# 0xPolygonZero/proof-protocol-decoder

Measured on AMD Instinct MI355X. Metric: txn-proofs/sec (whole node), 256-txn synthetic block, higher is better.
Workload: dtype u64 (Goldilocks field)

## Files before the change

### include/bpg.h

```cpp
#ifndef BPG_H
#define BPG_H
#include <stddef.h>
#include <stdint.h>

#ifdef __cplusplus
extern "C" {
#endif

typedef enum {
  BP_OK = 0,
  BP_ERR_ABORTED = -1,
  BP_ERR_INVALID_INPUT = -2,
  BP_ERR_RANGE = -3,
  BP_ERR_DEVICE = -4,
  BP_ERR_VERIFY = -5,
  BP_ERR_UNSUPPORTED = -6
} bp_status;

const char* bp_last_error(void);
const char* bp_version(void);
int bp_device_count(void);
int bp_use_blocking_sync(int device);
int bp_host_wait_mode(int device);

// ... 4 lines not shown
enum { BP_NTT_FWD_BR2NAT = 0, BP_NTT_INV_NAT2BR = 1, BP_NTT_FWD_NAT = 2, BP_NTT_INV_NAT = 3 };
int bp_ntt_batch(uint64_t* d_cols, uint32_t log_n, uint32_t n_cols, uint64_t col_stride, int dir,
                 void* stream);

int bp_intt_batch(const uint64_t* d_values, uint64_t in_stride, uint64_t* d_coeffs_out, uint64_t out_stride,
                  uint32_t log_n, uint32_t n_cols, void* stream);

int bp_lde_batch(const uint64_t* d_in, uint64_t in_stride, uint64_t* d_coeffs_out, uint64_t coeffs_stride,
                 uint64_t* d_lde_out, uint64_t lde_stride, uint32_t log_n, uint32_t rate_bits,
                 uint32_t n_cols, int from_coeffs, void* stream);

int bp_debug_copy_u64(const uint64_t* d_in, uint64_t* d_out, uint64_t n, void* stream);

int bp_debug_field_ops(const uint64_t* d_a, const uint64_t* d_b, uint64_t* d_out, uint64_t n, void* stream);
int bp_debug_lazy_forms(const uint64_t* d_a, const uint64_t* d_b, uint64_t* d_out, uint64_t n, void* stream);
int bp_debug_mul_pow2(const uint64_t* d_a, uint64_t* d_out, uint64_t n, void* stream);

void bp_tune_quad_threshold(uint64_t n_perms);
void bp_tune_merkle_fused(int mode);
void bp_tune_merkle_wide(int log2_parents);
void bp_tune_poseidon_mx(int on);
void bp_tune_poseidon_mx_sets(int sets);
void bp_tune_poseidon_grouped(int on);
void bp_tune_assume_loaded(int mode);
void bp_tune_rec_batch(int n);
void bp_tune_side_lanes(int n);
void bp_tune_rec_riders(int on);
void bp_tune_txn_group(int n);
void bp_tune_rec_group(int mode);
int bp_debug_rec_batch_histogram(uint64_t* out, uint32_t n, int reset);
// ... 343 lines not shown
```

### proof_protocol_decoder_amd/_abi.py

```python
import ctypes as C
from ctypes import POINTER as P

vp, cp, i, sz, dbl = C.c_void_p, C.c_char_p, C.c_int, C.c_size_t, C.c_double
u8, u32, u64, i32, i64 = C.c_uint8, C.c_uint32, C.c_uint64, C.c_int32, C.c_int64
u8p, u32p, u64p, i32p, szp = P(u8), P(u32), P(u64), P(i32), P(sz)
u8pp = P(u8p)

BP_OK, BP_ERR_ABORTED, BP_ERR_INVALID_INPUT, BP_ERR_RANGE, BP_ERR_DEVICE, BP_ERR_VERIFY, BP_ERR_UNSUPPORTED = 0, -1, -2, -3, -4, -5, -6
STATUS_NAMES = {v: k for k, v in list(globals().items()) if k == "BP_OK" or k.startswith("BP_ERR_")}
BP_SET_SKIP_LINK_CHECK = 1
BP_NUM_TABLES, BP_IR_WORDS, BP_PV_WORDS = 7, 25, 13

KNOBS = ("quad_threshold", "assume_loaded", "merkle_fused", "merkle_wide", "poseidon_mx", "poseidon_mx_sets",
         "poseidon_grouped", "ntt_mx", "ntt_split", "k5_spread", "host_wait", "host_poseidon", "rec_batch",
         "witness_threads", "side_lanes")


def _u32s(*names):
    return [(n, u32) for n in names]


class AirFamily(C.Structure):
    _fields_ = _u32s("first_index", "count", "kind", "degree")

# ... 105 lines not shown
_trace = (i, [vp, u64, u32, vp, vp])
_check = [u32, _cfg, vp, u64, vp, u64p, u32, u64p, u32p, P(AirViolation), u32, u32p]
_knob, _ir_flag, _buf = (None, [i]), (i, [u64p, i]), [u8pp, szp]
PROTOTYPES = {
    "bp_last_error": (cp, []),
    "bp_version": (cp, []),
    "bp_device_count": (i, []),
    "bp_use_blocking_sync": (i, [i]),
    "bp_host_wait_mode": (i, [i]),
    "bp_ntt_batch": (i, [vp, u32, u32, u64, i, vp]),
    "bp_intt_batch": (i, [vp, u64, vp, u64, u32, u32, vp]),
    "bp_lde_batch": (i, [vp, u64, vp, u64, vp, u64, u32, u32, u32, i, vp]),
    "bp_debug_copy_u64": (i, [vp, vp, u64, vp]),
    "bp_debug_field_ops": (i, [vp, vp, vp, u64, vp]),
    "bp_debug_lazy_forms": (i, [vp, vp, vp, u64, vp]),
    "bp_debug_mul_pow2": (i, [vp, vp, u64, vp]),
    "bp_tune_quad_threshold": (None, [u64]),
    "bp_tune_merkle_fused": _knob,
    "bp_tune_merkle_wide": _knob,
    "bp_tune_poseidon_mx": _knob,
    "bp_tune_poseidon_mx_sets": _knob,
    "bp_tune_poseidon_grouped": _knob,
    "bp_tune_assume_loaded": _knob,
    "bp_tune_rec_batch": _knob,
    "bp_tune_side_lanes": _knob,
    "bp_tune_rec_riders": _knob,
    "bp_tune_txn_group": _knob,
    "bp_tune_rec_group": _knob,
    "bp_debug_rec_batch_histogram": (i, [u64p, u32, i]),
    "bp_tune_witness_threads": _knob,
# ... 119 lines not shown
```

### proof_protocol_decoder_amd/csrc/air.hpp

```cpp
#pragma once
#include <cstdint>
#include <type_traits>
#include "gl.hpp"
#if defined(__HIP__)
#include "poseidon.cuh"
#endif

namespace bpg {
namespace air {

constexpr uint32_t SYNTHETIC = 0, KECCAK_F = 1, LOGIC = 2, MEMORY = 3, ARITHMETIC = 4, BYTE_PACKING = 5, KECCAK_SPONGE = 6, ARITHMETIC_MUL = 7, PLONK = 8, COUNT = 9;

struct Shape {
  uint32_t air_id, n_cols, n_const, deg_pow;
};

template <class T>
struct Ops;

#if defined(__HIP__)
template <>
struct Ops<uint64_t> {
  typedef uint64_t T;
  static __device__ __forceinline__ T k(uint64_t c) { return c; }
// ... 654 lines not shown
    out.all(U4 + k, F::sub(F::add(F::mul(m, conv), cin), F::add(p, F::mul(F::k(65536), c))));
    cin = c;
  }
  if (u == 7) out.all(U5, cin);
}
}

namespace plonk {
constexpr uint32_t N_COLS = 135, N_CONST = 85, N_ROUTED = 80, N_SLOTS = 20, N_SBOX = 11, N_CONSTRAINTS = 213, N_UNITS = 11;
constexpr uint32_t CST_ARITH = 0, CST_SBOX = 1, CST_C0 = 2, CST_C1 = 3, CST_HASH = 4, CST_SIGMA = 5;
constexpr uint32_t COL_SBOX = 80;
constexpr uint32_t G0 = 0, G1 = 20, G2 = 64, G3 = 86, G4 = 90, G5 = 208;
constexpr uint32_t HASH_ROW0 = 4, HASH_ROWS_MAX = 13, ZERO_ROW = 1, MAX_PI = 8 * HASH_ROWS_MAX;
constexpr uint32_t MERKLE_ROW0 = HASH_ROW0 + HASH_ROWS_MAX, MERKLE_ROWS_MAX = 96, MERKLE_ZERO_COL = 79, LEAF_ROWS_MAX = 120;
constexpr uint32_t H_IN = 0, H_OUT = 12, H_FULL1 = 24, H_PART = 60, H_FULL2 = 82, H_SWAP = 130, H_DELTA = 131, H_WIRES = 135;
struct Layout {
  uint32_t pi_len, n_paths, depth, path_pi0, leaf_len = 0;
};
GL_HD uint32_t hash_rows(uint32_t pi_len) { return (pi_len + 7) / 8; }
GL_HD uint32_t merkle_rows(const Layout& L) { return L.n_paths * L.depth; }
GL_HD uint32_t leaf_rows(const Layout& L) { return L.leaf_len ? L.n_paths * hash_rows(L.leaf_len) : 0; }
GL_HD uint32_t leaf_row0(const Layout& L) { return MERKLE_ROW0 + merkle_rows(L); }
GL_HD uint32_t arith_row0(const Layout& L) { return (MERKLE_ROW0 + merkle_rows(L) + leaf_rows(L) + 3) & ~3u; }
GL_HD bool layout_ok(const Layout& L, uint32_t n) {
  return L.pi_len >= 1 && L.pi_len <= MAX_PI && merkle_rows(L) <= MERKLE_ROWS_MAX && (L.n_paths == 0 || L.depth >= 1) &&
         L.path_pi0 + 8 * L.n_paths <= L.pi_len && (L.leaf_len == 0 || (L.leaf_len > 8 && L.n_paths >= 1)) &&
         leaf_rows(L) <= LEAF_ROWS_MAX && arith_row0(L) + 4 <= n;
}
GL_HD bool hash_word_is_carried(uint32_t pi_len, uint32_t h, uint32_t k) {
  const uint32_t H = hash_rows(pi_len), last = pi_len - 8 * (H - 1);
// ... 596 lines not shown
```

### proof_protocol_decoder_amd/csrc/prover.cpp

```cpp
#include <cstdio>
#include <cstdlib>
#include "prover.hpp"
#include "tune.hpp"
#include <algorithm>
#include <chrono>
#if defined(__x86_64__)
#include <immintrin.h>
#endif
#include <memory>
#include <mutex>
#include <unordered_map>
#include <thread>

namespace bpg {

static const uint64_t RC_HOST[360] = {
#include "poseidon_rc.inc"
};
static inline uint64_t sbox_host(uint64_t x) {
  uint64_t x2 = gl::mulc(x, x), x4 = gl::mulc(x2, x2), x3 = gl::mulc(x2, x);
  return gl::mulc(x3, x4);
}
static const uint32_t MDS_C[12] = {17, 15, 41, 16, 2, 28, 13, 13, 39, 18, 34, 20};
static inline void mds_finish_host(const uint64_t al[12], const uint64_t ah[12], uint64_t s[12]) {
// ... 514 lines not shown
                  int loaded, uint32_t batch) {
  QuotArgs& qa = *out;
  const uint32_t log_n = cfg.log_n, r = cfg.rate_bits, R = 1u << r, C = cfg.n_cols, K = cfg.n_const;
  const air::Shape shape{cfg.air_id, C, K, cfg.deg_pow};
  const uint32_t A = air::any_n_aux(shape);
  const uint64_t N = (uint64_t)1 << log_n, M = N << r;
  const uint64_t wM = gl::root(log_n + r), wN = gl::root(log_n);
  qa.trace_stride = qa.aux_stride = qa.const_stride = M;
  TRY(get_table(0, log_n, 0, &qa.tw_n));
  qa.air_id = cfg.air_id;
  qa.log_n = log_n; qa.rate_bits = r; qa.n_cols = C; qa.n_const = K; qa.n_aux = A; qa.deg_pow = cfg.deg_pow;
  qa.n_air_constraints = air::any_n_constraints(shape);
  qa.n_constraints = qa.n_air_constraints + air::any_n_ctl_constraints(shape);
  qa.side_rows = cfg.air_id == air::PLONK ? 1 : 0;
  qa.n_air_units = air::any_n_units(shape) - qa.side_rows;
  qa.aux_per_unit = cfg.air_id == air::SYNTHETIC ? std::max<uint32_t>(16, (A + 15) / 16) : A;
  qa.n_ctl_units = cfg.air_id == air::PLONK ? 0 : (A + qa.aux_per_unit - 1) / qa.aux_per_unit;
  qa.n_ports = air::prog::is_registered(cfg.air_id) && A > 1 ? A / 2 : 0;
  if (qa.n_ports) qa.n_ctl_units = qa.n_ports;
  const uint32_t n_units = qa.n_air_units + qa.n_ctl_units, wg_x = (uint32_t)((M + 255) / 256) * std::max<uint32_t>(1, batch);
  const uint32_t loaded_rows = (cfg.air_id == air::SYNTHETIC && !tune().k5_spread.load(std::memory_order_relaxed))
                                   ? 1 : std::min<uint32_t>(n_units, std::max<uint32_t>(1, (256 + wg_x - 1) / wg_x));
  const bool is_loaded = loaded < 0 ? device_loaded() : loaded != 0;
  const uint32_t want_rows = is_loaded ? loaded_rows : std::min<uint32_t>(n_units, std::max<uint32_t>(1, (2048 + wg_x - 1) / wg_x));
  qa.units_per_wg = (n_units + want_rows - 1) / want_rows;
  qa.alpha0 = alpha0; qa.alpha1 = alpha1;
  qa.g = wN; qa.g_inv = gl::inv(wN); qa.n_inv = gl::inv(N);
  if (coset)
    for (uint32_t t = 0; t < R; t++) {
      coset->g_t[t] = gl::mulc(gl::GENERATOR, gl::pow(wM, t));
// ... 414 lines not shown
```

### proof_protocol_decoder_amd/csrc/stark_api.cpp

```cpp
#include <algorithm>
#include <cstdlib>
#include <cstring>
#include <vector>
#include "caller_table.hpp"

using namespace bpg;

namespace {
constexpr uint32_t LONE_PI_LEN = 4;
void lone_public_input_list(uint64_t seed, uint64_t out[LONE_PI_LEN]) {
  for (uint64_t j = 0; j < LONE_PI_LEN; j++) {
    uint64_t z = (seed ^ ((0x50 + j) << 32)) + 0x9E3779B97F4A7C15ULL;
    z = (z ^ (z >> 30)) * 0xBF58476D1CE4E5B9ULL;
    z = (z ^ (z >> 27)) * 0x94D049BB133111EBULL;
    out[j] = gl::canon(z ^ (z >> 31));
  }
}
int prove_lone(Worker& w, const CallerTable& t, uint8_t** out, size_t* out_len) {
  Challenger ch;
  Committed consts, trace;
  const uint64_t* d_values = nullptr;
  int rc = commit_caller_table(w, ch, t, &consts, &trace, &d_values);
  if (rc) return rc;
  Ctl ctl;
// ... 3 lines not shown
  std::vector<uint64_t> proof;
  if ((rc = stark_prove(w, t.cfg, t.cfg.n_const ? &consts : nullptr, trace, d_values, ctl, ch, proof))) return rc;
  return emit(proof, out, out_len);
}
}

extern "C" {

void bp_free_buffer(uint8_t* buf) { std::free(buf); }
int bp_debug_poseidon_host(uint64_t* states, size_t n) try {
  if (!states && n) return bpg::fail(BP_ERR_INVALID_INPUT, "bp_debug_poseidon_host: null states");
  for (size_t i = 0; i < n; i++) bpg::poseidon_host(states + 12 * i);
  return BP_OK;
}
BPG_ABI_CATCH("bp_debug_poseidon_host")

void bp_release_cached_memory(void) { release_parked_workers(); }

int bp_stark_prove_air(uint32_t air_id, const bp_stark_cfg* cfg, uint64_t seed, uint64_t const_seed, int device,
                       uint8_t** out, size_t* out_len) try {
  if (!cfg || !out || !out_len) return fail(BP_ERR_INVALID_INPUT, "bp_stark_prove_air: null argument");
  if (air::prog::is_registered(air_id))
    return fail(BP_ERR_INVALID_INPUT, "bp_stark_prove_air: a registered AIR has no witness generator to draw from a seed: prove its trace "
                "with bp_stark_prove_trace");
  const StarkCfg c = to_cfg(*cfg, air_id);
  int rc = check_cfg(c);
  if (rc) return rc;
  const uint64_t N = (uint64_t)1 << c.log_n;
  WorkerLease lease(device, table_arena_bytes(c, false) + ARENA_SLACK);
  if (lease.rc()) return lease.rc();
// ... 415 lines not shown
```

### proof_protocol_decoder_amd/csrc/stark_kernels.hip

```cpp
#include "common.hpp"
#include "gl.hpp"
#include "poseidon.cuh"
#include "poseidon_mx.cuh"
#include "stark_kernels.hpp"
#include "arg_ring.hpp"
#include "quotient_dev.cuh"
#include "air_program.hpp"

namespace {

using gl::Ext;
using namespace bpg::k5;

__device__ __forceinline__ uint64_t splitmix64(uint64_t x) {
  uint64_t z = x + 0x9E3779B97F4A7C15ULL;
  z = (z ^ (z >> 30)) * 0xBF58476D1CE4E5B9ULL;
  z = (z ^ (z >> 27)) * 0x94D049BB133111EBULL;
  return z ^ (z >> 31);
}
__device__ __forceinline__ uint64_t rnd(uint64_t seed, uint64_t col, uint64_t row) {
  return gl::canon(splitmix64(seed ^ (col << 32) ^ row));
}
__device__ __forceinline__ uint64_t pow_e(uint64_t t, uint32_t e) {
  return e == 3 ? gl::mulc(gl::mulc(t, t), t) : t;
// ... 689 lines not shown
    aux[(uint64_t)(k + 1 < ct::PLONK_CHUNKS ? k + 1 : 0) * n] = P;
  }
}
__global__ void __launch_bounds__(256) plonk_partial_products_kernel(bpg::ArgPtr<bpg::AuxArgs> args, uint32_t log_n) {
  BPG_ARG_BATCH(bpg::AuxArgs, args);
  if (gridDim.x * gridDim.y * gridDim.z <= 64) __builtin_amdgcn_s_setprio(3);
  const bpg::AuxArgs& a = batch[blockIdx.z];
  const uint32_t n = 1u << log_n, i = blockIdx.x * blockDim.x + threadIdx.x, c = blockIdx.y / 9, k = 1 + blockIdx.y % 9;
  if (i >= n) return;
  const uint64_t z_next = a.aux[(uint64_t)(10 * c) * n + ((i + 1) & (n - 1))];
  uint64_t* p = a.aux + (uint64_t)(10 * c + k) * n + i;
  *p = gl::mulc(*p, z_next);
}

#ifndef BPG_PLONK_HASH_WAVES
#define BPG_PLONK_HASH_WAVES 2
#endif
template <uint32_t AIR>
__global__ void __launch_bounds__(256) __attribute__((amdgpu_waves_per_eu(AIR == bpg::air::KECCAK_F ? 3 : 1)))
quotient_air_kernel(bpg::ArgPtr<bpg::QuotArgs> args) {
  BPG_ARG_BATCH(bpg::QuotArgs, args);
  if (gridDim.x * gridDim.y * gridDim.z <= 64) __builtin_amdgcn_s_setprio(3);
  const bpg::QuotArgs& q = batch[blockIdx.z];
  const uint64_t rows = (uint64_t)1 << (q.log_n + q.rate_bits);
  const uint64_t pos = blockIdx.x * (uint64_t)blockDim.x + threadIdx.x;
  if (pos >= rows) return;
  const uint32_t n = 1u << q.log_n;
  const uint32_t t = (uint32_t)(pos >> q.log_n), m = (uint32_t)(pos & (n - 1));
  DevEmit out{q.apow, q.n_constraints, row_point(q, t, m),
              {gl::dot_zero(), gl::dot_zero(), gl::dot_zero(), gl::dot_zero()}, 0, 0, false};
  DevRow row{q.trace_lde, q.aux_lde, q.const_lde, q.trace_stride, q.aux_stride, q.const_stride, pos,
// ... 9 lines not shown
      const uint32_t k0 = (u - q.n_air_units) * q.aux_per_unit, k1 = min(k0 + q.aux_per_unit, q.n_aux);
      const bpg::air::Shape cs{AIR, q.n_cols, q.n_const, q.deg_pow};
      bpg::air::ctl::eval<uint64_t>(cs, q.n_air_constraints, k0, k1, q.ctl.v, row, out);
    }
  }
  const uint64_t r0 = out.result(0), r1 = out.result(1);
  if (gridDim.y == 1 && q.side_rows == 0) {
    const uint64_t zh_inv = q.apow[2 * (size_t)q.n_constraints + 32 + t];
    q.qvals[pos] = gl::mulc(r0, zh_inv);
    q.qvals[rows + pos] = gl::mulc(r1, zh_inv);
  } else {
    q.partial[((uint64_t)blockIdx.y * 2) * rows + pos] = r0;
    q.partial[((uint64_t)blockIdx.y * 2 + 1) * rows + pos] = r1;
  }
}
__global__ void __launch_bounds__(256) __attribute__((amdgpu_waves_per_eu(BPG_PLONK_HASH_WAVES)))
quotient_plonk_hash_kernel(bpg::ArgPtr<bpg::QuotArgs> args, uint32_t wg_row) {
  BPG_ARG_BATCH(bpg::QuotArgs, args);
  if (gridDim.x * gridDim.y * gridDim.z <= 64) __builtin_amdgcn_s_setprio(3);
  const bpg::QuotArgs& q = batch[blockIdx.z];
  const uint64_t rows = (uint64_t)1 << (q.log_n + q.rate_bits);
  const uint64_t pos = blockIdx.x * (uint64_t)blockDim.x + threadIdx.x;
  if (pos >= rows) return;
  const uint32_t n = 1u << q.log_n;
  const uint32_t t = (uint32_t)(pos >> q.log_n), m = (uint32_t)(pos & (n - 1));
  DevEmit out{q.apow, q.n_constraints, row_point(q, t, m),
              {gl::dot_zero(), gl::dot_zero(), gl::dot_zero(), gl::dot_zero()}, 0, 0, false};
  DevRow row{q.trace_lde, q.aux_lde, q.const_lde, q.trace_stride, q.aux_stride, q.const_stride, pos,
             ((uint64_t)t << q.log_n) | ((m + 1) & (n - 1)), out.rp.x, q.ctl.pub};
  bpg::air::plonk::eval_hash_unit<uint64_t, DevRow, DevEmit, false>(row, out);
  const uint64_t qh = row.cst(bpg::air::plonk::CST_HASH);
  q.partial[((uint64_t)wg_row * 2) * rows + pos] = gl::mulc(out.result(0), qh);
  q.partial[((uint64_t)wg_row * 2 + 1) * rows + pos] = gl::mulc(out.result(1), qh);
}
__global__ void __launch_bounds__(256) quotient_sum_kernel(bpg::ArgPtr<bpg::QuotArgs> args, uint32_t n_wg_rows) {
  BPG_ARG_BATCH(bpg::QuotArgs, args);
  if (gridDim.x * gridDim.y * gridDim.z <= 64) __builtin_amdgcn_s_setprio(3);
  const bpg::QuotArgs& q = batch[blockIdx.z];
  const uint64_t rows = (uint64_t)1 << (q.log_n + q.rate_bits);
  const uint64_t pos = blockIdx.x * (uint64_t)blockDim.x + threadIdx.x;
  if (pos >= rows) return;
  const uint32_t j = blockIdx.y, t = (uint32_t)(pos >> q.log_n);
  uint64_t acc = 0;
  for (uint32_t c = 0; c < n_wg_rows; c++) acc = gl::addc(acc, q.partial[((uint64_t)c * 2 + j) * rows + pos]);
  q.qvals[(uint64_t)j * rows + pos] = gl::mulc(acc, q.apow[2 * (size_t)q.n_constraints + 32 + t]);
}
struct CosetTab {
  uint64_t v[48];
};
struct AlphaTabArgs {
  uint64_t* out;
  uint64_t a0, a1;
};
__global__ void __launch_bounds__(256)
alpha_table_kernel(bpg::ArgPtr<AlphaTabArgs> args, uint32_t T, CosetTab ct) {
  BPG_ARG_BATCH(AlphaTabArgs, args);
  if (gridDim.x * gridDim.y * gridDim.z <= 64) __builtin_amdgcn_s_setprio(3);
  uint64_t* __restrict__ out = batch[blockIdx.z].out;
  const uint64_t a0 = batch[blockIdx.z].a0, a1 = batch[blockIdx.z].a1;
  const uint32_t e = blockIdx.x * blockDim.x + threadIdx.x;
  if (blockIdx.y == 0 && e < 48) out[2 * (uint64_t)T + e] = ct.v[e];
  if (e >= T) return;
  out[(uint64_t)blockIdx.y * T + e] = gl::pow(blockIdx.y ? a1 : a0, e);
}
__global__ void __launch_bounds__(256) quotient_chunks_kernel(bpg::ArgPtr<bpg::ChunkArgs> args) {
  BPG_ARG_BATCH(bpg::ChunkArgs, args);
  if (gridDim.x * gridDim.y * gridDim.z <= 64) __builtin_amdgcn_s_setprio(3);
  const bpg::ChunkArgs& c = batch[blockIdx.z];
  const uint32_t pos = blockIdx.x * blockDim.x + threadIdx.x, n = 1u << c.log_n;
  if (pos >= n) return;
  const uint32_t j = blockIdx.y, R = 1u << c.rate_bits;
  const uint64_t* e = c.e + (uint64_t)j * ((uint64_t)n << c.rate_bits);
  uint64_t d[16];
  for (uint32_t t = 0; t < R; t++) d[t] = gl::mulc(e[(uint64_t)t * n + pos], c.inv_scale[(uint64_t)t * n + pos]);
// ... 633 lines not shown
    BPG_LAUNCH_CHECK();
    plonk_partial_products_kernel<<<dim3(gx, 18, batch), 256, 0, st>>>(ab, log_n);
    BPG_LAUNCH_CHECK();
    return BP_OK;
  }
  const dim3 grid(n_aux - p0, 1, batch);
  const uint32_t reads = air_id < air::COUNT ? air::DESC[air_id].aux_reads : 0;
  KernelTimer kt(PROF_AUX, st, 8.0 * (double)((uint64_t)1 << log_n) * (reads + 1) * (n_aux - p0) * batch, true);
  air::dispatch(reads ? air_id : air::ARITHMETIC, [&](auto A) {
    if constexpr (air::DESC[A.value].aux_reads || A.value == air::ARITHMETIC)
      BPG_LAUNCH_TIMED(kt, aux_suffix_product_kernel<A.value>, grid, threads, 0, st, ab, log_n, n_cols);
  });
  BPG_LAUNCH_CHECK();
  return BP_OK;
}
int launch_quotient(const QuotArgs* qs, uint32_t batch, const QuotCoset& coset, hipStream_t st) {
  if (int rc = check_batch(batch)) return rc;
  const QuotArgs& q = qs[0];
  const uint64_t rows = (uint64_t)1 << (q.log_n + q.rate_bits);
  CosetTab ct;
  for (int t = 0; t < 16; t++) { ct.v[t] = coset.g_t[t]; ct.v[16 + t] = coset.zh_t[t]; ct.v[32 + t] = coset.zh_inv_t[t]; }
  AlphaTabArgs tabs[MAX_LOCKSTEP];
  for (uint32_t b = 0; b < batch; b++) tabs[b] = AlphaTabArgs{const_cast<uint64_t*>(qs[b].apow), qs[b].alpha0, qs[b].alpha1};
  BPG_ARG_BLOCKS(at, tabs, batch, st);
  alpha_table_kernel<<<dim3(ceil_div(q.n_constraints, 256), 2, batch), 256, 0, st>>>(at, q.n_constraints, ct);
  BPG_LAUNCH_CHECK();
  const uint32_t n_units = q.n_air_units + q.n_ctl_units, wg_rows = ceil_div(n_units, q.units_per_wg);
  BPG_ARG_BLOCKS(qb, qs, batch, st);
  if (q.n_ports)
    if (int rc = launch_beta_tables(qb_dev, batch, st)) return rc;
  dim3 g1(ceil_div(rows, 256), wg_rows, batch);
  KernelTimer kt(PROF_K5 + (q.air_id < air::COUNT ? q.air_id : 0), st, 8.0 * (double)rows * ((double)q.n_cols + q.n_aux + q.n_const + 2) * batch, true);
  if (bpg::air::prog::is_registered(q.air_id)) {
    if (int rc = launch_quotient_program(qb_dev, q, g1, kt, st)) return rc;
  } else air::dispatch(q.air_id, [&](auto A) { BPG_LAUNCH_TIMED(kt, quotient_air_kernel<A.value>, g1, 256, 0, st, qb); });
  kt.stop();
  if (q.side_rows) {
    BPG_LAUNCH_CHECK();
    KernelTimer kh(PROF_K5 + q.air_id, st, 0.0, true);
    BPG_LAUNCH_TIMED(kh, quotient_plonk_hash_kernel, dim3(ceil_div(rows, 256), 1, batch), 256, 0, st, qb, wg_rows);
  }
// ... 153 lines not shown
```

### proof_protocol_decoder_amd/csrc/stark_kernels.hpp

```cpp
#pragma once
#include <hip/hip_runtime.h>
#include <cstdint>
#include "air.hpp"
#include "gl.hpp"

namespace bpg {

struct Ctl {
  uint64_t v[4];
  uint64_t pub[4] = {0, 0, 0, 0};
};

constexpr uint32_t MAX_BATCH = 8;
constexpr uint32_t MAX_LOCKSTEP = 24;
int arg_ring_put(hipStream_t st, const void* blocks, size_t bytes, const void** dev);
template <class A>
using ArgPtr = const __attribute__((address_space(4))) A*;
template <class A>
inline ArgPtr<A> arg_ptr(const A* dev) { return (ArgPtr<A>)dev; }
#define BPG_ARG_BATCH(T, args) const T* __restrict__ batch = (const T*)(args)
template <class A>
inline int arg_put(hipStream_t st, const A* a, uint32_t n, const A** dev) {
  const void* d = nullptr;
  const int rc = arg_ring_put(st, a, sizeof(A) * n, &d);
// ... 2 lines not shown
}

struct QuotArgs {
  const uint64_t *trace_lde, *aux_lde, *const_lde;
  uint64_t trace_stride, aux_stride, const_stride;
  uint64_t *partial, *qvals;
  const uint64_t* tw_n;
  const uint64_t* apow;
  uint32_t air_id, log_n, rate_bits, n_cols, n_const, n_aux, deg_pow;
  uint32_t n_air_constraints, n_constraints, n_air_units, n_ctl_units, aux_per_unit, units_per_wg;
  uint32_t side_rows;
  uint32_t n_ports;
  uint64_t alpha0, alpha1, g, g_inv, n_inv;
  Ctl ctl;
};
inline size_t quotient_table_words(const QuotArgs& q) { return 2 * (size_t)q.n_constraints + 48 + (q.n_ports ? 256 : 0); }
struct QuotCoset {
  uint64_t g_t[16], zh_t[16], zh_inv_t[16];
};
struct SynthTraceArgs {
  uint64_t* trace;
  const uint64_t* consts;
  uint64_t seed;
};
struct AuxArgs {
  const uint64_t* trace;
  uint64_t* aux;
  Ctl ctl;
  const uint64_t* consts = nullptr;
};
struct PowerVecArgs {
// ... 116 lines not shown
int launch_aux(const AuxArgs* a, uint32_t batch, uint32_t air_id, uint32_t n_cols, uint32_t log_n, hipStream_t st);
int launch_plonk_constants(uint64_t* d_out, uint32_t log_n, uint64_t seed, const air::plonk::Layout& lay, hipStream_t st);
struct PlonkTraceArgs {
  uint64_t* trace;
  const uint64_t* consts;
  uint64_t seed, pub[4];
  const uint64_t* hash_rows;
  uint32_t n_hash_rows;
  uint32_t n_merkle_rows = 0, arith_row0 = (air::plonk::MERKLE_ROW0 + 3) & ~3u;
};
int launch_plonk_trace(const PlonkTraceArgs* a, uint32_t batch, uint32_t log_n, hipStream_t st);
int launch_quotient(const QuotArgs* q, uint32_t batch, const QuotCoset& coset, hipStream_t st);
inline int launch_quotient(const QuotArgs& q, const QuotCoset& coset, hipStream_t st) { return launch_quotient(&q, 1, coset, st); }
struct KernelTimer;
int launch_quotient_program(const QuotArgs* qb, const QuotArgs& q0, dim3 grid, KernelTimer& kt, hipStream_t st);
int launch_beta_tables(const QuotArgs* qb, uint32_t batch, hipStream_t st);
int launch_port_terms(const AuxArgs& a, uint32_t air_id, uint32_t log_n, uint64_t trace_stride, uint64_t* d_pole, hipStream_t st);
int launch_port_products(const AuxArgs* a, uint32_t batch, uint32_t air_id, uint32_t log_n, uint64_t trace_stride, hipStream_t st);
int launch_quotient_chunks(const ChunkArgs* c, uint32_t batch, hipStream_t st);
int launch_power_vectors(const PowerVecArgs* a, uint32_t batch, uint32_t log_n, uint32_t n_points, hipStream_t st);
inline int launch_power_vectors(uint64_t* d_out, uint32_t log_n, gl::Ext z0, gl::Ext z1, uint32_t n_points,
                                hipStream_t st, gl::Ext z2 = gl::Ext{1, 0}) {
  const PowerVecArgs a{d_out, {z0, z1, z2}};
  return launch_power_vectors(&a, 1, log_n, n_points, st);
}
int launch_alpha_pows(const AlphaPowArgs* a, uint32_t batch, uint32_t count, hipStream_t st);
int launch_openings(const uint64_t* d_coeffs, uint64_t stride, uint32_t log_n, uint32_t n_cols,
                    const uint64_t* d_pw, uint32_t n_points, uint64_t* d_out, hipStream_t st);
int launch_openings_multi(const OpenMulti* m, uint32_t batch, hipStream_t st);
int launch_combine_partial_multi(const CombineMulti* m, uint32_t batch, uint32_t total_chunks, hipStream_t st);
// ... 29 lines not shown
```

### proof_protocol_decoder_amd/ops.py

```python
import contextlib
import ctypes as C

import numpy as np
import torch

from ._lib import KNOBS, StarkCfg, call_for_buffer, check, lib, own

NTT_FWD_BR2NAT, NTT_INV_NAT2BR, NTT_FWD_NAT, NTT_INV_NAT = 0, 1, 2, 3


def _stream():
    return torch.cuda.current_stream().cuda_stream


_tuned_active = False


@contextlib.contextmanager
def tuned(**knobs):
    global _tuned_active
    if _tuned_active:
        raise RuntimeError("ops.tuned() inside ops.tuned(): name all the knobs in one call")
    unknown = sorted(set(knobs) - set(KNOBS))
    if unknown:
# ... 56 lines not shown
def field_ops(a, b):
    _require_cuda(a)
    _require_cuda(b)
    n = a.numel()
    out = torch.empty((15, n), dtype=torch.int64, device=a.device)
    check(own().bp_debug_field_ops(a.data_ptr(), b.data_ptr(), out.data_ptr(), n, _stream()))
    return out


def lazy_forms(a, b):
    _require_cuda(a)
    _require_cuda(b)
    n = a.numel()
    out = torch.empty((12, n), dtype=torch.int64, device=a.device)
    check(own().bp_debug_lazy_forms(a.data_ptr(), b.data_ptr(), out.data_ptr(), n, _stream()))
    return out


def mul_pow2(a):
    _require_cuda(a)
    n = a.numel()
    out = torch.empty((21, n), dtype=torch.int64, device=a.device)
    check(own().bp_debug_mul_pow2(a.data_ptr(), out.data_ptr(), n, _stream()))
    return out


AIR_SYNTHETIC, AIR_KECCAK_F = 0, 1
KECCAK_COLS = 2431
LOGIC_COLS = 524
MEMORY_COLS = 45
# ... 447 lines not shown
```

Baseline: 38.97.

## Fold Poseidon gate constraints into precomputed linear weights for the PLONK hash quotient

```diff
diff --git a/include/bpg.h b/include/bpg.h
--- a/include/bpg.h
+++ b/include/bpg.h
@@ -42,6 +42,8 @@
 
 int bp_debug_field_ops(const uint64_t* d_a, const uint64_t* d_b, uint64_t* d_out, uint64_t n, void* stream);
 int bp_debug_lazy_forms(const uint64_t* d_a, const uint64_t* d_b, uint64_t* d_out, uint64_t n, void* stream);
+int bp_debug_plonk_hash_fold(const uint64_t alphas[2], uint64_t* d_out, void* stream);
+int bp_debug_plonk_hash_fold_host(const uint64_t alphas[2], uint64_t* out);
 int bp_debug_mul_pow2(const uint64_t* d_a, uint64_t* d_out, uint64_t n, void* stream);
 
 void bp_tune_quad_threshold(uint64_t n_perms);
diff --git a/proof_protocol_decoder_amd/_abi.py b/proof_protocol_decoder_amd/_abi.py
--- a/proof_protocol_decoder_amd/_abi.py
+++ b/proof_protocol_decoder_amd/_abi.py
@@ -143,6 +143,8 @@
     "bp_debug_copy_u64": (i, [vp, vp, u64, vp]),
     "bp_debug_field_ops": (i, [vp, vp, vp, u64, vp]),
     "bp_debug_lazy_forms": (i, [vp, vp, vp, u64, vp]),
+    "bp_debug_plonk_hash_fold": (i, [u64p, vp, vp]),
+    "bp_debug_plonk_hash_fold_host": (i, [u64p, u64p]),
     "bp_debug_mul_pow2": (i, [vp, vp, u64, vp]),
     "bp_tune_quad_threshold": (None, [u64]),
     "bp_tune_merkle_fused": _knob,
diff --git a/proof_protocol_decoder_amd/csrc/air.hpp b/proof_protocol_decoder_amd/csrc/air.hpp
--- a/proof_protocol_decoder_amd/csrc/air.hpp
+++ b/proof_protocol_decoder_amd/csrc/air.hpp
@@ -692,6 +692,7 @@
 constexpr uint32_t HASH_ROW0 = 4, HASH_ROWS_MAX = 13, ZERO_ROW = 1, MAX_PI = 8 * HASH_ROWS_MAX;
 constexpr uint32_t MERKLE_ROW0 = HASH_ROW0 + HASH_ROWS_MAX, MERKLE_ROWS_MAX = 96, MERKLE_ZERO_COL = 79, LEAF_ROWS_MAX = 120;
 constexpr uint32_t H_IN = 0, H_OUT = 12, H_FULL1 = 24, H_PART = 60, H_FULL2 = 82, H_SWAP = 130, H_DELTA = 131, H_WIRES = 135;
+constexpr uint32_t HASH_FOLD_PAIRS = 118, HASH_FOLD_WORDS = 2 * HASH_FOLD_PAIRS + 2;
 struct Layout {
   uint32_t pi_len, n_paths, depth, path_pi0, leaf_len = 0;
 };
diff --git a/proof_protocol_decoder_amd/csrc/plonk_hash_fold.hpp b/proof_protocol_decoder_amd/csrc/plonk_hash_fold.hpp
--- /dev/null
+++ b/proof_protocol_decoder_amd/csrc/plonk_hash_fold.hpp
@@ -0,0 +1,101 @@
+#pragma once
+#include <cstdint>
+#include <vector>
+#include "air.hpp"
+#include "gl.hpp"
+
+namespace bpg {
+namespace air {
+namespace plonk {
+
+inline uint32_t hash_fold_pair_full(uint32_t r, uint32_t i) {
+  return r == 0 ? 106 + i : r <= 3 ? 12 * (r - 1) + i : 58 + 12 * (r - 26) + i;
+}
+inline uint32_t hash_fold_pair_part(uint32_t r) { return 36 + (r - 4); }
+
+inline void hash_fold_weights(const uint64_t (&A)[HASH_FOLD_PAIRS], uint64_t (&C)[HASH_FOLD_PAIRS], uint64_t& K) {
+  auto mds_t = [](const uint64_t (&g)[12], uint64_t (&h)[12]) {
+    for (uint32_t c = 0; c < 12; c++) {
+      uint64_t acc = 0;
+      for (uint32_t r = 0; r < 12; r++) acc = gl::addc(acc, gl::mulc(poseidon_mds_entry(r, c), g[r]));
+      h[c] = acc;
+    }
+  };
+  auto dot_rc = [](const uint64_t (&g)[12], uint32_t r) {
+    uint64_t acc = 0;
+    for (uint32_t i = 0; i < 12; i++) acc = gl::addc(acc, gl::mulc(g[i], poseidon_rc(12 * r + i)));
+    return acc;
+  };
+  K = 0;
+  uint64_t g[12], h[12];
+  auto full = [&](uint32_t k0, int rc_round, uint32_t sigma_round) {
+    for (uint32_t i = 0; i < 12; i++) g[i] = A[k0 + i];
+    mds_t(g, h);
+    for (uint32_t i = 0; i < 12; i++) C[hash_fold_pair_full(sigma_round, i)] = h[i];
+    if (rc_round >= 0) K = gl::addc(K, dot_rc(g, (uint32_t)rc_round));
+  };
+  for (uint32_t r = 1; r <= 3; r++) full(12 * (r - 1), (int)r, r - 1);
+  for (uint32_t r = 27; r <= 29; r++) full(58 + 12 * (r - 26), (int)r, r - 1);
+  full(106, -1, 29);
+  for (uint32_t i = 0; i < 12; i++) g[i] = A[58 + i];
+  K = gl::addc(K, dot_rc(g, 26));
+  for (uint32_t r = 25; r >= 4; r--) {
+    mds_t(g, h);
+    C[hash_fold_pair_part(r)] = h[0];
+    for (uint32_t i = 0; i < 12; i++) g[i] = h[i];
+    g[0] = A[hash_fold_pair_part(r)];
+    K = gl::addc(K, dot_rc(g, r));
+  }
+  mds_t(g, h);
+  for (uint32_t i = 0; i < 12; i++) C[hash_fold_pair_full(3, i)] = h[i];
+}
+
+inline void hash_fold_block_host(uint32_t T, uint64_t alpha0, uint64_t alpha1, uint64_t (&out)[HASH_FOLD_WORDS]) {
+  for (uint32_t j = 0; j < 2; j++) {
+    uint64_t A[HASH_FOLD_PAIRS], C[HASH_FOLD_PAIRS], K;
+    for (uint32_t p = 0; p < HASH_FOLD_PAIRS; p++) A[p] = gl::pow(j ? alpha1 : alpha0, T - 1 - G4 - p);
+    hash_fold_weights(A, C, K);
+    for (uint32_t p = 0; p < HASH_FOLD_PAIRS; p++) out[2 * p + j] = gl::negc(C[p]);
+    out[2 * HASH_FOLD_PAIRS + j] = K;
+  }
+}
+
+constexpr uint32_t HASH_FOLD_BLOCKS = 3, HASH_FOLD_OUTPUTS = HASH_FOLD_PAIRS + 1, HASH_FOLD_PIECE_TERMS = 4;
+constexpr uint32_t HASH_FOLD_COEF0 = 2 * 256 * HASH_FOLD_BLOCKS;
+constexpr uint32_t HASH_FOLD_T_MIN = G4 + HASH_FOLD_PAIRS, HASH_FOLD_T_MAX = 256;
+inline std::vector<uint64_t> hash_fold_table() {
+  std::vector<uint64_t> col((size_t)HASH_FOLD_PAIRS * HASH_FOLD_OUTPUTS);
+  for (uint32_t k = 0; k < HASH_FOLD_PAIRS; k++) {
+    uint64_t A[HASH_FOLD_PAIRS] = {}, C[HASH_FOLD_PAIRS], K;
+    A[k] = 1;
+    hash_fold_weights(A, C, K);
+    for (uint32_t p = 0; p < HASH_FOLD_PAIRS; p++) col[(size_t)k * HASH_FOLD_OUTPUTS + p] = C[p];
+    col[(size_t)k * HASH_FOLD_OUTPUTS + HASH_FOLD_PAIRS] = K;
+  }
+  std::vector<uint64_t> tab(HASH_FOLD_COEF0 + 256 * HASH_FOLD_BLOCKS * HASH_FOLD_PIECE_TERMS, 0);
+  uint32_t block = 0, piece = 0, output = 0;
+  for (uint32_t o = 0; o < HASH_FOLD_OUTPUTS; o++) {
+    uint32_t lo = HASH_FOLD_PAIRS, hi = 0;
+    for (uint32_t k = 0; k < HASH_FOLD_PAIRS; k++)
+      if (col[(size_t)k * HASH_FOLD_OUTPUTS + o]) {
+        if (lo == HASH_FOLD_PAIRS) lo = k;
+        hi = k;
+      }
+    if (lo == HASH_FOLD_PAIRS) return {};
+    const uint32_t n = (hi - lo + HASH_FOLD_PIECE_TERMS) / HASH_FOLD_PIECE_TERMS;
+    if (piece + n > 256) { block++; piece = output = 0; }
+    if (block >= HASH_FOLD_BLOCKS || n > 255) return {};
+    tab[256 * HASH_FOLD_BLOCKS + 256 * block + output++] = (uint64_t)n | (uint64_t)piece << 8 | (uint64_t)o << 16;
+    for (uint32_t k0 = lo; k0 <= hi; k0 += HASH_FOLD_PIECE_TERMS) {
+      const uint32_t k1 = k0 + HASH_FOLD_PIECE_TERMS - 1 < hi ? k0 + HASH_FOLD_PIECE_TERMS - 1 : hi;
+      for (uint32_t k = k0; k <= k1; k++)
+        tab[HASH_FOLD_COEF0 + HASH_FOLD_PIECE_TERMS * (256 * block + piece) + (k - k0)] = col[(size_t)k * HASH_FOLD_OUTPUTS + o];
+      tab[256 * block + piece++] = (uint64_t)(k1 - k0 + 1) | (uint64_t)k0 << 8;
+    }
+  }
+  return tab;
+}
+
+}
+}
+}
diff --git a/proof_protocol_decoder_amd/csrc/prover.cpp b/proof_protocol_decoder_amd/csrc/prover.cpp
--- a/proof_protocol_decoder_amd/csrc/prover.cpp
+++ b/proof_protocol_decoder_amd/csrc/prover.cpp
@@ -552,6 +552,10 @@
   qa.n_constraints = qa.n_air_constraints + air::any_n_ctl_constraints(shape);
   qa.side_rows = cfg.air_id == air::PLONK ? 1 : 0;
   qa.n_air_units = air::any_n_units(shape) - qa.side_rows;
+  if (qa.side_rows) {
+    const uint64_t* fold = nullptr;
+    TRY(get_hash_fold_table(&fold));
+  }
   qa.aux_per_unit = cfg.air_id == air::SYNTHETIC ? std::max<uint32_t>(16, (A + 15) / 16) : A;
   qa.n_ctl_units = cfg.air_id == air::PLONK ? 0 : (A + qa.aux_per_unit - 1) / qa.aux_per_unit;
   qa.n_ports = air::prog::is_registered(cfg.air_id) && A > 1 ? A / 2 : 0;
diff --git a/proof_protocol_decoder_amd/csrc/stark_api.cpp b/proof_protocol_decoder_amd/csrc/stark_api.cpp
--- a/proof_protocol_decoder_amd/csrc/stark_api.cpp
+++ b/proof_protocol_decoder_amd/csrc/stark_api.cpp
@@ -3,6 +3,7 @@
 #include <cstring>
 #include <vector>
 #include "caller_table.hpp"
+#include "plonk_hash_fold.hpp"
 
 using namespace bpg;
 
@@ -41,6 +42,26 @@
   return BP_OK;
 }
 BPG_ABI_CATCH("bp_debug_poseidon_host")
+
+static int hash_fold_alphas(const char* who, const uint64_t alphas[2], const void* out) {
+  if (!alphas || !out) return bpg::fail(BP_ERR_INVALID_INPUT, "%s: null argument", who);
+  if (alphas[0] >= gl::P || alphas[1] >= gl::P) return bpg::fail(BP_ERR_INVALID_INPUT, "%s: non-canonical alpha", who);
+  return BP_OK;
+}
+int bp_debug_plonk_hash_fold(const uint64_t alphas[2], uint64_t* d_out, void* stream) try {
+  if (int rc = hash_fold_alphas("bp_debug_plonk_hash_fold", alphas, d_out)) return rc;
+  if (int rc = init_ntt_kernels()) return rc;
+  return debug_plonk_hash_fold(alphas[0], alphas[1], d_out, as_stream(stream));
+}
+BPG_ABI_CATCH("bp_debug_plonk_hash_fold")
+int bp_debug_plonk_hash_fold_host(const uint64_t alphas[2], uint64_t* out) try {
+  if (int rc = hash_fold_alphas("bp_debug_plonk_hash_fold_host", alphas, out)) return rc;
+  uint64_t block[air::plonk::HASH_FOLD_WORDS];
+  air::plonk::hash_fold_block_host(air::plonk::N_CONSTRAINTS + air::ctl::PLONK_N_CONSTRAINTS, alphas[0], alphas[1], block);
+  std::memcpy(out, block, sizeof(block));
+  return BP_OK;
+}
+BPG_ABI_CATCH("bp_debug_plonk_hash_fold_host")
 
 void bp_release_cached_memory(void) { release_parked_workers(); }
 
diff --git a/proof_protocol_decoder_amd/csrc/stark_kernels.hip b/proof_protocol_decoder_amd/csrc/stark_kernels.hip
--- a/proof_protocol_decoder_amd/csrc/stark_kernels.hip
+++ b/proof_protocol_decoder_amd/csrc/stark_kernels.hip
@@ -1,3 +1,6 @@
+#include <map>
+#include <mutex>
+#include <vector>
 #include "common.hpp"
 #include "gl.hpp"
 #include "poseidon.cuh"
@@ -6,6 +9,7 @@
 #include "arg_ring.hpp"
 #include "quotient_dev.cuh"
 #include "air_program.hpp"
+#include "plonk_hash_fold.hpp"
 
 namespace {
 
@@ -727,7 +731,7 @@
 }
 
 #ifndef BPG_PLONK_HASH_WAVES
-#define BPG_PLONK_HASH_WAVES 2
+#define BPG_PLONK_HASH_WAVES 4
 #endif
 template <uint32_t AIR>
 __global__ void __launch_bounds__(256) __attribute__((amdgpu_waves_per_eu(AIR == bpg::air::KECCAK_F ? 3 : 1)))
@@ -767,6 +771,99 @@
     q.partial[((uint64_t)blockIdx.y * 2 + 1) * rows + pos] = r1;
   }
 }
+struct HashFoldWeights {
+  const uint64_t* a;
+  const uint64_t* nc;
+  uint32_t T;
+};
+template <int N>
+__device__ __forceinline__ void hash_fold_pairs(const uint64_t (&wire)[N], uint64_t (&x)[N], const HashFoldWeights& fw,
+                                                uint32_t p0, gl::DotAcc (&acc)[4]) {
+  __builtin_amdgcn_sched_barrier(0);
+  poseidon::sbox_n<N>(x);
+  __builtin_amdgcn_sched_barrier(0);
+#pragma unroll
+  for (int i = 0; i < N; i++) {
+    const uint64_t *ap = fw.a - (p0 + i), *k = fw.nc + 2 * (size_t)(p0 + i);
+    const uint64_t a[4] = {wire[i], wire[i], x[i], x[i]};
+    const uint64_t w[4] = {ap[0], ap[fw.T], k[0], k[1]};
+    gl::dot_mad4(acc, a, w);
+  }
+}
+template <int N>
+__device__ __forceinline__ void hash_fold_wires(const DevRow& row, uint32_t col0, const HashFoldWeights& fw, uint32_t p0,
+                                                gl::DotAcc (&acc)[4]) {
+  uint64_t wire[N], x[N];
+#pragma unroll
+  for (int i = 0; i < N; i++) wire[i] = x[i] = row.loc(col0 + i);
+  hash_fold_pairs<N>(wire, x, fw, p0, acc);
+}
+__device__ __forceinline__ void eval_hash_fold(const DevRow& row, const uint64_t* __restrict__ apow, uint32_t T,
+                                               uint64_t& r0, uint64_t& r1) {
+  namespace pk = bpg::air::plonk;
+  typedef bpg::air::Ops<uint64_t> F;
+  typedef bpg::air::PoseidonOps<uint64_t> H;
+  const HashFoldWeights fw{apow + (T - 1 - pk::G4), apow + 2 * (size_t)T + 48, T};
+  gl::DotAcc acc[4] = {gl::dot_zero(), gl::dot_zero(), gl::dot_zero(), gl::dot_zero()};
+  {
+    const uint64_t sw = row.loc(pk::H_SWAP);
+    uint64_t lhs[4], rhs[4], dl[4], pr[4], g[4], d[4];
+#pragma unroll
+    for (uint32_t i = 0; i < 4; i++) {
+      lhs[i] = row.loc(pk::H_IN + i);
+      rhs[i] = row.loc(pk::H_IN + 4 + i);
+      dl[i] = row.loc(pk::H_DELTA + i);
+      pr[i] = F::sub(rhs[i], lhs[i]);
+    }
+    const uint64_t s4[4] = {sw, sw, sw, sw};
+    F::mul4(s4, pr, g);
+#pragma unroll
+    for (uint32_t i = 0; i < 4; i++) d[i] = F::sub(dl[i], g[i]);
+    const uint64_t bit = F::mul(sw, F::sub(sw, F::k(1)));
+    const uint64_t* a0 = apow + (T - 1 - pk::G5 - 4);
+    const uint64_t* a1 = a0 + T;
+    {
+      const uint64_t a[4] = {d[0], d[0], d[1], d[1]}, w[4] = {a0[3], a1[3], a0[2], a1[2]};
+      gl::dot_mad4(acc, a, w);
+    }
+    {
+      const uint64_t a[4] = {d[2], d[2], d[3], d[3]}, w[4] = {a0[1], a1[1], a0[0], a1[0]};
+      gl::dot_mad4(acc, a, w);
+    }
+    {
+      const uint64_t a[4] = {bit, bit, 0, 0}, w[4] = {a0[4], a1[4], 0, 0};
+      gl::dot_mad4(acc, a, w);
+    }
+    uint64_t wire[4], x[4];
+#pragma unroll
+    for (uint32_t i = 0; i < 4; i++) {
+      wire[i] = row.loc(pk::H_OUT + i);
+      x[i] = H::add_rc0(F::add(lhs[i], dl[i]), i);
+    }
+    hash_fold_pairs<4>(wire, x, fw, 106, acc);
+#pragma unroll
+    for (uint32_t i = 0; i < 4; i++) {
+      wire[i] = row.loc(pk::H_OUT + 4 + i);
+      x[i] = H::add_rc0(F::sub(rhs[i], dl[i]), 4 + i);
+    }
+    hash_fold_pairs<4>(wire, x, fw, 110, acc);
+#pragma unroll
+    for (uint32_t i = 0; i < 4; i++) {
+      wire[i] = row.loc(pk::H_OUT + 8 + i);
+      x[i] = H::add_rc0(row.loc(pk::H_IN + 8 + i), 8 + i);
+    }
+    hash_fold_pairs<4>(wire, x, fw, 114, acc);
+  }
+  constexpr uint32_t N4 = 25;
+  static_assert(pk::H_SWAP - pk::H_FULL1 == 4 * N4 + 6 && pk::HASH_FOLD_PAIRS == 118, "the pair layout of plonk_hash_fold.hpp");
+#pragma unroll 1
+  for (uint32_t g = 0; g < N4; g++) hash_fold_wires<4>(row, pk::H_FULL1 + 4 * g, fw, 4 * g, acc);
+  hash_fold_wires<3>(row, pk::H_FULL1 + 4 * N4, fw, 4 * N4, acc);
+  hash_fold_wires<3>(row, pk::H_FULL1 + 4 * N4 + 3, fw, 4 * N4 + 3, acc);
+  const uint64_t* K = fw.nc + 2 * pk::HASH_FOLD_PAIRS;
+  r0 = gl::subc(gl::addc(gl::dot_reduce(acc[0]), gl::dot_reduce(acc[2])), K[0]);
+  r1 = gl::subc(gl::addc(gl::dot_reduce(acc[1]), gl::dot_reduce(acc[3])), K[1]);
+}
 __global__ void __launch_bounds__(256) __attribute__((amdgpu_waves_per_eu(BPG_PLONK_HASH_WAVES)))
 quotient_plonk_hash_kernel(bpg::ArgPtr<bpg::QuotArgs> args, uint32_t wg_row) {
   BPG_ARG_BATCH(bpg::QuotArgs, args);
@@ -775,16 +872,12 @@
   const uint64_t rows = (uint64_t)1 << (q.log_n + q.rate_bits);
   const uint64_t pos = blockIdx.x * (uint64_t)blockDim.x + threadIdx.x;
   if (pos >= rows) return;
-  const uint32_t n = 1u << q.log_n;
-  const uint32_t t = (uint32_t)(pos >> q.log_n), m = (uint32_t)(pos & (n - 1));
-  DevEmit out{q.apow, q.n_constraints, row_point(q, t, m),
-              {gl::dot_zero(), gl::dot_zero(), gl::dot_zero(), gl::dot_zero()}, 0, 0, false};
-  DevRow row{q.trace_lde, q.aux_lde, q.const_lde, q.trace_stride, q.aux_stride, q.const_stride, pos,
-             ((uint64_t)t << q.log_n) | ((m + 1) & (n - 1)), out.rp.x, q.ctl.pub};
-  bpg::air::plonk::eval_hash_unit<uint64_t, DevRow, DevEmit, false>(row, out);
+  DevRow row{q.trace_lde, q.aux_lde, q.const_lde, q.trace_stride, q.aux_stride, q.const_stride, pos, pos, 0, q.ctl.pub};
+  uint64_t r0, r1;
+  eval_hash_fold(row, q.apow, q.n_constraints, r0, r1);
   const uint64_t qh = row.cst(bpg::air::plonk::CST_HASH);
-  q.partial[((uint64_t)wg_row * 2) * rows + pos] = gl::mulc(out.result(0), qh);
-  q.partial[((uint64_t)wg_row * 2 + 1) * rows + pos] = gl::mulc(out.result(1), qh);
+  q.partial[((uint64_t)wg_row * 2) * rows + pos] = gl::mulc(r0, qh);
+  q.partial[((uint64_t)wg_row * 2 + 1) * rows + pos] = gl::mulc(r1, qh);
 }
 __global__ void __launch_bounds__(256) quotient_sum_kernel(bpg::ArgPtr<bpg::QuotArgs> args, uint32_t n_wg_rows) {
   BPG_ARG_BATCH(bpg::QuotArgs, args);
@@ -806,11 +899,42 @@
   uint64_t a0, a1;
 };
 __global__ void __launch_bounds__(256)
-alpha_table_kernel(bpg::ArgPtr<AlphaTabArgs> args, uint32_t T, CosetTab ct) {
+alpha_table_kernel(bpg::ArgPtr<AlphaTabArgs> args, uint32_t T, CosetTab ct, const uint64_t* __restrict__ fold) {
   BPG_ARG_BATCH(AlphaTabArgs, args);
   if (gridDim.x * gridDim.y * gridDim.z <= 64) __builtin_amdgcn_s_setprio(3);
   uint64_t* __restrict__ out = batch[blockIdx.z].out;
   const uint64_t a0 = batch[blockIdx.z].a0, a1 = batch[blockIdx.z].a1;
+  if (fold) {
+    namespace pk = bpg::air::plonk;
+    __shared__ uint64_t pw[256], part[256];
+    const uint32_t l = threadIdx.x, j = blockIdx.y, e0 = T - 1 - pk::G4;
+    const uint32_t lane = 256 * blockIdx.x + l;
+    const uint64_t piece = fold[lane], o = fold[256 * pk::HASH_FOLD_BLOCKS + lane];
+    uint64_t coef[pk::HASH_FOLD_PIECE_TERMS];
+#pragma unroll
+    for (uint32_t i = 0; i < pk::HASH_FOLD_PIECE_TERMS; i++) coef[i] = fold[pk::HASH_FOLD_COEF0 + pk::HASH_FOLD_PIECE_TERMS * lane + i];
+    const uint64_t p = l < T ? gl::pow(j ? a1 : a0, l) : 0;
+    pw[l] = p;
+    if (blockIdx.x == 0) {
+      if (j == 0 && l < 48) out[2 * (uint64_t)T + l] = ct.v[l];
+      if (l < T) out[(uint64_t)j * T + l] = p;
+    }
+    __syncthreads();
+    const uint32_t terms = (uint32_t)piece & 0xff, k0 = (uint32_t)(piece >> 8) & 0xff;
+    uint64_t acc = 0;
+#pragma unroll
+    for (uint32_t i = 0; i < pk::HASH_FOLD_PIECE_TERMS; i++)
+      if (i < terms) acc = gl::addc(acc, gl::mulc(coef[i], pw[e0 - k0 - i]));
+    part[l] = acc;
+    __syncthreads();
+    const uint32_t pieces = (uint32_t)o & 0xff, first = (uint32_t)(o >> 8) & 0xff, slot = (uint32_t)(o >> 16);
+    if (!pieces) return;
+    uint64_t sum = 0;
+    for (uint32_t i = 0; i < pieces; i++) sum = gl::addc(sum, part[first + i]);
+    uint64_t* __restrict__ w = out + 2 * (uint64_t)T + 48;
+    w[2 * slot + j] = slot < pk::HASH_FOLD_PAIRS ? gl::negc(sum) : sum;
+    return;
+  }
   const uint32_t e = blockIdx.x * blockDim.x + threadIdx.x;
   if (blockIdx.y == 0 && e < 48) out[2 * (uint64_t)T + e] = ct.v[e];
   if (e >= T) return;
@@ -1474,17 +1598,64 @@
   BPG_LAUNCH_CHECK();
   return BP_OK;
 }
+int get_hash_fold_table(const uint64_t** out) {
+  static std::mutex mu;
+  static std::map<int, const uint64_t*> tabs;
+  int dev = 0;
+  BPG_HIP(hipGetDevice(&dev));
+  std::lock_guard<std::mutex> lk(mu);
+  auto it = tabs.find(dev);
+  if (it == tabs.end()) {
+    static const std::vector<uint64_t> host = air::plonk::hash_fold_table();
+    if (host.empty()) return fail(BP_ERR_DEVICE, "the Poseidon gate's fold table does not fit its workgroups");
+    uint64_t* d = nullptr;
+    BPG_HIP(hipMalloc(reinterpret_cast<void**>(&d), host.size() * 8));
+    BPG_HIP(hipMemcpy(d, host.data(), host.size() * 8, hipMemcpyHostToDevice));
+    it = tabs.emplace(dev, d).first;
+  }
+  *out = it->second;
+  return BP_OK;
+}
+static int launch_alpha_tables(const QuotArgs* qs, uint32_t batch, const QuotCoset& coset, hipStream_t st) {
+  const QuotArgs& q = qs[0];
+  CosetTab ct;
+  for (int t = 0; t < 16; t++) { ct.v[t] = coset.g_t[t]; ct.v[16 + t] = coset.zh_t[t]; ct.v[32 + t] = coset.zh_inv_t[t]; }
+  const uint64_t* fold = nullptr;
+  if (q.side_rows) {
+    if (q.n_constraints < air::plonk::HASH_FOLD_T_MIN || q.n_constraints > air::plonk::HASH_FOLD_T_MAX)
+      return fail(BP_ERR_INVALID_INPUT, "the Poseidon gate's fold weights are made for a constraint list of %u..%u entries, not %u",
+                  air::plonk::HASH_FOLD_T_MIN, air::plonk::HASH_FOLD_T_MAX, q.n_constraints);
+    if (int rc = get_hash_fold_table(&fold)) return rc;
+  }
+  AlphaTabArgs tabs[MAX_LOCKSTEP];
+  for (uint32_t b = 0; b < batch; b++) tabs[b] = AlphaTabArgs{const_cast<uint64_t*>(qs[b].apow), qs[b].alpha0, qs[b].alpha1};
+  BPG_ARG_BLOCKS(at, tabs, batch, st);
+  alpha_table_kernel<<<dim3(fold ? air::plonk::HASH_FOLD_BLOCKS : ceil_div(q.n_constraints, 256), 2, batch), 256, 0, st>>>(at, q.n_constraints, ct, fold);
+  BPG_LAUNCH_CHECK();
+  return BP_OK;
+}
+int debug_plonk_hash_fold(uint64_t alpha0, uint64_t alpha1, uint64_t* d_out, hipStream_t st) {
+  QuotArgs q{};
+  q.n_constraints = air::plonk::N_CONSTRAINTS + air::ctl::PLONK_N_CONSTRAINTS;
+  q.side_rows = 1;
+  q.alpha0 = alpha0; q.alpha1 = alpha1;
+  struct Table {
+    uint64_t* d = nullptr;
+    ~Table() { (void)hipFree(d); }
+  } tab;
+  BPG_HIP(hipMalloc(reinterpret_cast<void**>(&tab.d), quotient_table_words(q) * 8));
+  q.apow = tab.d;
+  if (int rc = launch_alpha_tables(&q, 1, QuotCoset{}, st)) return rc;
+  BPG_HIP(hipMemcpyAsync(d_out, tab.d + 2 * (size_t)q.n_constraints + 48, air::plonk::HASH_FOLD_WORDS * 8, hipMemcpyDeviceToDevice, st));
+  BPG_HIP(hipStreamSynchronize(st));
+  return BP_OK;
+}
 int launch_quotient(const QuotArgs* qs, uint32_t batch, const QuotCoset& coset, hipStream_t st) {
   if (int rc = check_batch(batch)) return rc;
   const QuotArgs& q = qs[0];
   const uint64_t rows = (uint64_t)1 << (q.log_n + q.rate_bits);
-  CosetTab ct;
-  for (int t = 0; t < 16; t++) { ct.v[t] = coset.g_t[t]; ct.v[16 + t] = coset.zh_t[t]; ct.v[32 + t] = coset.zh_inv_t[t]; }
-  AlphaTabArgs tabs[MAX_LOCKSTEP];
-  for (uint32_t b = 0; b < batch; b++) tabs[b] = AlphaTabArgs{const_cast<uint64_t*>(qs[b].apow), qs[b].alpha0, qs[b].alpha1};
-  BPG_ARG_BLOCKS(at, tabs, batch, st);
-  alpha_table_kernel<<<dim3(ceil_div(q.n_constraints, 256), 2, batch), 256, 0, st>>>(at, q.n_constraints, ct);
-  BPG_LAUNCH_CHECK();
+  if (q.n_ports && q.side_rows) return fail(BP_ERR_INVALID_INPUT, "launch_quotient: lookup ports and a side row in one table");
+  if (int rc = launch_alpha_tables(qs, batch, coset, st)) return rc;
   const uint32_t n_units = q.n_air_units + q.n_ctl_units, wg_rows = ceil_div(n_units, q.units_per_wg);
   BPG_ARG_BLOCKS(qb, qs, batch, st);
   if (q.n_ports)
diff --git a/proof_protocol_decoder_amd/csrc/stark_kernels.hpp b/proof_protocol_decoder_amd/csrc/stark_kernels.hpp
--- a/proof_protocol_decoder_amd/csrc/stark_kernels.hpp
+++ b/proof_protocol_decoder_amd/csrc/stark_kernels.hpp
@@ -40,7 +40,9 @@
   uint64_t alpha0, alpha1, g, g_inv, n_inv;
   Ctl ctl;
 };
-inline size_t quotient_table_words(const QuotArgs& q) { return 2 * (size_t)q.n_constraints + 48 + (q.n_ports ? 256 : 0); }
+inline size_t quotient_table_words(const QuotArgs& q) {
+  return 2 * (size_t)q.n_constraints + 48 + (q.n_ports ? 256 : 0) + (q.side_rows ? air::plonk::HASH_FOLD_WORDS : 0);
+}
 struct QuotCoset {
   uint64_t g_t[16], zh_t[16], zh_inv_t[16];
 };
@@ -187,6 +189,8 @@
 inline int launch_quotient(const QuotArgs& q, const QuotCoset& coset, hipStream_t st) { return launch_quotient(&q, 1, coset, st); }
 struct KernelTimer;
 int launch_quotient_program(const QuotArgs* qb, const QuotArgs& q0, dim3 grid, KernelTimer& kt, hipStream_t st);
+int get_hash_fold_table(const uint64_t** out);
+int debug_plonk_hash_fold(uint64_t alpha0, uint64_t alpha1, uint64_t* d_out, hipStream_t st);
 int launch_beta_tables(const QuotArgs* qb, uint32_t batch, hipStream_t st);
 int launch_port_terms(const AuxArgs& a, uint32_t air_id, uint32_t log_n, uint64_t trace_stride, uint64_t* d_pole, hipStream_t st);
 int launch_port_products(const AuxArgs* a, uint32_t batch, uint32_t air_id, uint32_t log_n, uint64_t trace_stride, hipStream_t st);
diff --git a/proof_protocol_decoder_amd/ops.py b/proof_protocol_decoder_amd/ops.py
--- a/proof_protocol_decoder_amd/ops.py
+++ b/proof_protocol_decoder_amd/ops.py
@@ -94,6 +94,22 @@
     n = a.numel()
     out = torch.empty((12, n), dtype=torch.int64, device=a.device)
     check(own().bp_debug_lazy_forms(a.data_ptr(), b.data_ptr(), out.data_ptr(), n, _stream()))
+    return out
+
+
+PLONK_HASH_FOLD_WORDS = 2 * 118 + 2
+
+
+def plonk_hash_fold(alphas, device="cuda"):
+    out = torch.empty(PLONK_HASH_FOLD_WORDS, dtype=torch.int64, device=device)
+    check(own().bp_debug_plonk_hash_fold((C.c_uint64 * 2)(*[int(x) for x in alphas]), out.data_ptr(), _stream()))
+    return out
+
+
+def plonk_hash_fold_host(alphas):
+    out = np.zeros(PLONK_HASH_FOLD_WORDS, dtype=np.uint64)
+    check(own().bp_debug_plonk_hash_fold_host((C.c_uint64 * 2)(*[int(x) for x in alphas]),
+                                              out.ctypes.data_as(C.POINTER(C.c_uint64))))
     return out
 
 
```

Result: faster. 39.70, median of 6 (+1.9%).
